# duanzhiihao/myDetection

Hardware: AMD Instinct MI355X
Metric: images/sec at batch 32, 640x640, YOLOv3-80 (backbone -> FPN -> head -> decode -> NMS) (higher is better)
Workload: dtype f32; 1 GPU; yolov3_80 (Darknet-53 + YOLOv3 FPN/head + decode + conf 0.005/top-512/NMS 0.45), batch 32/GPU, 640x640, random-init calibrated weights, hipGraph replay (1 batch lane per GPU); global_batch=32, image_size=640, parallelism=dp1, batch_lanes=1, batch_lanes_rule=model.batch_lanes_hint, passes=153, exchange=none

## Files before the change

include/mydet.h:

```cpp
#ifndef MYDET_H
#define MYDET_H

#include <stdint.h>

#ifdef __cplusplus
extern "C" {
#endif

#define MYDET_ABI_VERSION 2

#define MYDET_E_BADARG   (-1)
#define MYDET_E_UNSUPP   (-2)

#define MYDET_ACT_NONE   0
#define MYDET_ACT_LEAKY  1
#define MYDET_ACT_SWISH  2

int mydet_abi_version(void);

int mydet_conv2d_igemm_f32(const float *x, int64_t ldx, const float *w,
                           const float *scale, const float *shift,
                           const float *residual, int64_t ldr, const float *a_gate,
                           void *workspace, int64_t workspace_bytes,
                           float *y, int64_t ldy,
// ... 36 lines not shown

int mydet_maxpool3s2_f32(const float *x, int64_t ldx, float *y, int64_t ldy, int B, int H, int W, int C,
                         int Ho, int Wo, void *stream);

int mydet_bifpn_fuse_f32(int n, const float *in0, int64_t ld0, int mode0, const float *in1, int64_t ld1, int mode1,
                         const float *in2, int64_t ld2, int mode2, const float *weights, float *y, int64_t ldy,
                         int B, int H, int W, int C, void *stream);

int mydet_upsample_concat_f32(const float *a, int64_t lda, int Ha, int Wa, int C1,
                              const float *b, int64_t ldb, int C2,
                              float *y, int64_t ldy, int B, int Ho, int Wo, void *stream);

int mydet_conv1x1_upcat_f32(const float *x_lo, int64_t ld_lo, int C_lo, const float *x_hi, int64_t ld_hi, int C_hi,
                            const float *w, const float *scale, const float *shift, void *workspace,
                            int64_t workspace_bytes, float *y, int64_t ldy, int B, int H, int W, int Cout, int act,
                            void *stream);

int64_t mydet_split_bf16_elems(int Cout, int K);
int mydet_split_bf16_f32(const float *w, int Cout, int K, uint16_t *planes, void *stream);
int mydet_conv2d_igemm_b3_f32(const float *x, int64_t ldx, const uint16_t *w_planes, const float *scale, const float *shift,
                              const float *residual, int64_t ldr, const float *a_gate, void *workspace, int64_t workspace_bytes, float *y,
                              int64_t ldy, int B, int H, int W, int Cin, int Cout, int KH, int KW, int stride, int pad_t,
                              int pad_l, int Ho, int Wo, int act, void *stream);
int mydet_conv3x3_p3_f32(const float *x, int64_t ldx, const uint16_t *w_planes, const float *scale, const float *shift,
                         const float *residual, int64_t ldr, float *y, int64_t ldy, int B, int H, int W, int Cin, int Cout,
                         int stride, int act, void *stream);
int mydet_conv3x3_p3_plan(int Ho, int Wo, int Cout, int stride, int32_t *out);
int mydet_conv_stem_p3_f32(const float *x, int64_t sxb, int64_t sxc, int64_t sxh, int64_t sxw, const uint16_t *w0_planes,
                           const float *scale0, const float *shift0, int act0, const uint16_t *w1_planes, const float *scale1,
                           const float *shift1, int act1, float *y, int64_t ldy, int B, int H, int W, int C0, int Cout,
                           int stride0, int pad_t, int pad_l, int Hs, int Ws, int stride1, void *stream);
int mydet_conv_stem_p3_lds_bytes(void);
int mydet_conv_b3_reload_tuning(void);

int mydet_conv_igemm_occupancy(int cfg, int *assumed);

int mydet_conv_igemm_plan(int cfg, int B, int Ho, int Wo, int Cin, int Cout, int taps,
                          int64_t workspace_bytes, int cus, int32_t *out);

int mydet_space_to_depth_f32(const float *x, int64_t sb, int64_t sc, int64_t sh, int64_t sw, float *y, int64_t ldy,
                             int B, int C, int H, int W, void *stream);

int mydet_spp_concat_f32(const float *x, int64_t ldx, float *y, int64_t ldy, int B, int H, int W, int C, int k0, int k1,
                         int k2, void *stream);

#define MYDET_DECODE_YOLO   0
#define MYDET_DECODE_RETINA 1
#define MYDET_DECODE_FCOS   2
#define MYDET_DECODE_RAPID  3
typedef struct mydet_decode_level {
    const float *box; int64_t ldbox;
    const float *cls; int64_t ldcls;
    const float *anchors_wh;
    int H, W;
    float stride;
    int64_t n_off;
} mydet_decode_level;
int mydet_decode_levels_f32(int mode, int nlevels, const mydet_decode_level *levels, int box_astride, int box_c0,
                            int cls_astride, int cls_c0, int conf_c0, int A, int C, int B, int img_h, int img_w,
                            float *bbox, int64_t *class_idx, float *score, int64_t N, void *stream);
int mydet_decode_uv5_levels_f32(int nlevels, const mydet_decode_level *levels, int box_astride, int box_c0,
                                int cls_astride, int cls_c0, int conf_c0, int A, int C, int B, int img_h, int img_w,
                                float *bbox, int64_t *class_idx, float *score, int64_t N, void *stream);
int mydet_decode_f32(int mode,
                     const float *box, int64_t ldbox, int box_astride, int box_c0,
                     const float *cls, int64_t ldcls, int cls_astride, int cls_c0, int conf_c0,
// ... 225 lines not shown
```

mydetection_amd/_lib.py:

```python
import ctypes
import os

_HERE = os.path.dirname(os.path.abspath(__file__))
LIB_PATH = os.environ.get('MYDET_LIB_PATH') or os.path.join(_HERE, 'lib', 'libmydet_hip.so')

c_int, c_i64, c_f32, c_f64, c_ptr = ctypes.c_int, ctypes.c_int64, ctypes.c_float, ctypes.c_double, ctypes.c_void_p

SIGNATURES = {
    'mydet_abi_version': [],
    'mydet_conv2d_igemm_f32': [c_ptr, c_i64, c_ptr, c_ptr, c_ptr, c_ptr, c_i64, c_ptr, c_ptr, c_i64, c_ptr, c_i64]
    + [c_int] * 13 + [c_ptr],
    'mydet_wino_weights_floats': [c_int, c_int],
    'mydet_wino_weights_f32': [c_ptr, c_int, c_int, c_ptr, c_ptr],
    'mydet_conv2d_wino_f32': [c_ptr, c_i64, c_ptr, c_ptr, c_ptr, c_ptr, c_i64, c_ptr, c_i64, c_ptr, c_i64] + [c_int] * 6
    + [c_ptr],
    'mydet_wino_plan': [c_int] * 5 + [c_i64, c_int, c_ptr],
    'mydet_wino4_weights_floats': [c_int, c_int],
    'mydet_wino4_weights_f32': [c_ptr, c_int, c_int, c_ptr, c_ptr],
    'mydet_wino4_workspace_bytes': [c_int, c_int, c_int, c_int, c_int],
    'mydet_wino4_reload_tuning': [],
    'mydet_conv_b3_reload_tuning': [],
    'mydet_conv_igemm_occupancy': [c_int, c_ptr],
    'mydet_conv_igemm_plan': [c_int] * 7 + [c_i64, c_int, c_ptr],
    'mydet_split_bf16_elems': [c_int, c_int],
    'mydet_split_bf16_f32': [c_ptr, c_int, c_int, c_ptr, c_ptr],
    'mydet_conv2d_igemm_b3_f32': [c_ptr, c_i64, c_ptr, c_ptr, c_ptr, c_ptr, c_i64, c_ptr, c_ptr, c_i64, c_ptr, c_i64] + [c_int] * 13 + [c_ptr],
    'mydet_conv3x3_p3_f32': [c_ptr, c_i64, c_ptr, c_ptr, c_ptr, c_ptr, c_i64, c_ptr, c_i64] + [c_int] * 7 + [c_ptr],
    'mydet_conv3x3_p3_plan': [c_int, c_int, c_int, c_int, c_ptr],
    'mydet_conv_stem_p3_f32': [c_ptr, c_i64, c_i64, c_i64, c_i64, c_ptr, c_ptr, c_ptr, c_int, c_ptr, c_ptr, c_ptr, c_int, c_ptr, c_i64]
    + [c_int] * 11 + [c_ptr],
    'mydet_conv_stem_p3_lds_bytes': [],
    'mydet_wino4_tail_plan': [c_int, c_int, c_int, c_int, c_int, c_int, c_ptr],
    'mydet_conv2d_wino4_f32': [c_ptr, c_i64, c_ptr, c_ptr, c_ptr, c_ptr, c_i64, c_ptr, c_i64, c_ptr, c_i64] + [c_int] * 6 + [c_ptr],
    'mydet_dwconv_slices': [c_int, c_int, c_int, c_int, c_int],
    'mydet_dwconv_se_groups': [c_int, c_int, c_int, c_int, c_int],
    'mydet_dwconv_f32': [c_ptr, c_i64, c_ptr, c_ptr, c_ptr, c_ptr, c_i64] + [c_int] * 11 + [c_ptr, c_int, c_ptr, c_ptr],
    'mydet_channel_sums_f32': [c_ptr, c_i64, c_int, c_int, c_int, c_int, c_ptr, c_int, c_ptr],
    'mydet_se_gate_f32': [c_ptr, c_int, c_int, c_int, c_int, c_ptr, c_ptr, c_int, c_ptr, c_ptr, c_ptr, c_ptr],
    'mydet_maxpool3s2_f32': [c_ptr, c_i64, c_ptr, c_i64] + [c_int] * 6 + [c_ptr],
    'mydet_bifpn_fuse_f32': [c_int, c_ptr, c_i64, c_int, c_ptr, c_i64, c_int, c_ptr, c_i64, c_int, c_ptr, c_ptr, c_i64,
                             c_int, c_int, c_int, c_int, c_ptr],
    'mydet_conv2d_stem_f32': [c_ptr, c_i64, c_i64, c_i64, c_i64, c_ptr, c_ptr, c_ptr, c_ptr, c_i64] + [c_int] * 10 + [c_ptr],
    'mydet_upsample_concat_f32': [c_ptr, c_i64, c_int, c_int, c_int, c_ptr, c_i64, c_int, c_ptr, c_i64, c_int, c_int,
                                  c_int, c_ptr],
    'mydet_conv1x1_upcat_f32': [c_ptr, c_i64, c_int, c_ptr, c_i64, c_int, c_ptr, c_ptr, c_ptr, c_ptr, c_i64, c_ptr, c_i64]
    + [c_int] * 5 + [c_ptr],
    'mydet_space_to_depth_f32': [c_ptr, c_i64, c_i64, c_i64, c_i64, c_ptr, c_i64, c_int, c_int, c_int, c_int, c_ptr],
    'mydet_spp_concat_f32': [c_ptr, c_i64, c_ptr, c_i64] + [c_int] * 7 + [c_ptr],
    'mydet_decode_levels_f32': [c_int, c_int, c_ptr, c_int, c_int, c_int, c_int, c_int, c_int, c_int, c_int, c_int, c_int,
                                c_ptr, c_ptr, c_ptr, c_i64, c_ptr],
    'mydet_decode_uv5_levels_f32': [c_int, c_ptr, c_int, c_int, c_int, c_int, c_int, c_int, c_int, c_int, c_int, c_int,
                                    c_ptr, c_ptr, c_ptr, c_i64, c_ptr],
    'mydet_decode_f32': [c_int, c_ptr, c_i64, c_int, c_int, c_ptr, c_i64, c_int, c_int, c_int, c_ptr, c_int, c_int,
                         c_int, c_int, c_int, c_f32, c_int, c_int, c_ptr, c_ptr, c_ptr, c_i64, c_i64, c_ptr],
# ... 168 lines not shown
```

mydetection_amd/csrc/common.h:

```cpp
#pragma once
#include <hip/hip_runtime.h>
#include <stdint.h>

#include "mydet.h"

typedef float f32x4 __attribute__((ext_vector_type(4)));
typedef float f32x16 __attribute__((ext_vector_type(16)));

#define MYDET_WAVE 64

static inline int mydet_launch_status() { return (int)hipGetLastError(); }

static inline int mydet_cu_count() {
    static int n = 0;
    if (n == 0) {
        int dev = 0, v = 0;
        if (hipGetDevice(&dev) == hipSuccess && hipDeviceGetAttribute(&v, hipDeviceAttributeMultiprocessorCount, dev) == hipSuccess && v > 0)
            n = v;
        else
            n = 256;
    }
    return n;
}

// ... 24 lines not shown
    return __builtin_amdgcn_rcpf(1.0f + __builtin_amdgcn_exp2f(t));
}

__device__ __forceinline__ float mydet_act(float v, int act) {
    if (act == MYDET_ACT_LEAKY) return v > 0.0f ? v : v * 0.1f;
    if (act == MYDET_ACT_SWISH) return v * mydet_sigmoid_fast(v);
    return v;
}

__device__ __forceinline__ void mydet_lds_barrier() {
    __builtin_amdgcn_fence(__ATOMIC_RELEASE, "workgroup", "local");
    __builtin_amdgcn_s_barrier();
    __builtin_amdgcn_fence(__ATOMIC_ACQUIRE, "workgroup", "local");
}

__device__ __forceinline__ __amdgpu_buffer_rsrc_t mydet_rsrc(const void *base, int64_t bytes) {
    const uint64_t a = (uint64_t)base;
    const unsigned lo = __builtin_amdgcn_readfirstlane((unsigned)a);
    const unsigned hi = __builtin_amdgcn_readfirstlane((unsigned)(a >> 32));
    const int64_t capped = bytes > 0x7FFFFFF0ll ? 0x7FFFFFF0ll : bytes;
    const int n = __builtin_amdgcn_readfirstlane((int)capped);
    return __builtin_amdgcn_make_buffer_rsrc((void *)(((uint64_t)hi << 32) | lo), 0, n, 0x00020000);
}

__device__ __forceinline__ int mydet_xcd_remap(int bid, int nblk) {
    const int xcd = bid & 7, q = nblk >> 3, r = nblk & 7;
    const int base = xcd < r ? xcd * (q + 1) : r * (q + 1) + (xcd - r) * q;
    return base + (bid >> 3);
}

int mydet_pw_skinny(const float *x, int64_t ldx, const float *w, const float *scale, const float *shift,
                    const float *residual, int64_t ldr, const float *gate, float *y, int64_t ldy, int B, int HW, int Cin,
                    int Cout, int act, void *stream);
```

mydetection_amd/csrc/conv_igemm.hip:

```cpp
#include <cstdlib>

#include "common.h"
#include "split_bf16.h"

namespace {

constexpr unsigned OOB = 0xFFFFFFFFu;

struct ConvArgs {
    const float *x, *w, *scale, *shift, *res, *gate;
    float *y;
    int64_t ldx, ldr, ldy;
    int B, H, W, Cin, Cout, KH, KW, stride, pad_t, pad_l, Ho, Wo, act;
    int M, K, ntiles, nblk;
    int tile0, splits;
    float *ws;
    size_t ws_bytes;
    const float *x1;
    int64_t ldx1;
    int C1;
    const unsigned short *wsplit;
};

typedef unsigned u32x4 __attribute__((ext_vector_type(4)));

__device__ __forceinline__ f32x4 buf_load16(__amdgpu_buffer_rsrc_t rsrc, unsigned voff) {
    return __builtin_bit_cast(f32x4, __builtin_amdgcn_raw_buffer_load_b128(rsrc, voff, 0, 0));
}

template <int ACT, bool RES, bool FULL, int TM, int TN>
__device__ __forceinline__ void epilogue(const ConvArgs &p, f32x16 (&acc)[TM][TN], int m_base, int n_base,
                                         int fr, int fh, const float (&pscl)[TN], const float (&psft)[TN]) {
    const __amdgpu_buffer_rsrc_t yr = mydet_rsrc(p.y, (int64_t)p.M * p.ldy * 4);
    const __amdgpu_buffer_rsrc_t rr = mydet_rsrc(RES ? p.res : p.y, (int64_t)p.M * (RES ? p.ldr : p.ldy) * 4);
    const unsigned ldy4 = (unsigned)p.ldy * 4u, ldr4 = (unsigned)p.ldr * 4u;
#pragma unroll
    for (int j = 0; j < TN; ++j) {
        const int n = n_base + j * 32 + fr;
        const bool nok = FULL || n < p.Cout;
        const float scl = pscl[j], sft = psft[j];
#pragma unroll
        for (int i = 0; i < TM; ++i) {
            const int mrow = m_base + i * 32 + 4 * fh;
            const unsigned ybase = (unsigned)mrow * ldy4 + (unsigned)n * 4u;
            const unsigned rbase = (unsigned)mrow * ldr4 + (unsigned)n * 4u;
            float rv[16];
            if (RES) {
#pragma unroll
                for (int r = 0; r < 16; ++r) {
                    const int dr = (r & 3) + 8 * (r >> 2);
                    const bool ok = FULL || (nok && mrow + dr < p.M);
                    rv[r] = __builtin_bit_cast(float, __builtin_amdgcn_raw_buffer_load_b32(
                                                          rr, ok ? rbase + (unsigned)dr * ldr4 : OOB, 0, 0));
                }
            }
#pragma unroll
            for (int r = 0; r < 16; ++r) {
                const int dr = (r & 3) + 8 * (r >> 2);
                float v = acc[i][j][r] * scl + sft;
                if (ACT == MYDET_ACT_LEAKY) v = v > 0.0f ? v : v * 0.1f;
                if (ACT == MYDET_ACT_SWISH) v = v * mydet_sigmoid_fast(v);
                if (RES) v += rv[r];
                const bool ok = FULL || (nok && mrow + dr < p.M);
                __builtin_amdgcn_raw_buffer_store_b32(__builtin_bit_cast(unsigned, v), yr,
                                                      ok ? ybase + (unsigned)dr * ldy4 : OOB, 0, 0);
            }
        }
    }
}

template <int BM, int BN, int WM, int WN, int BK, bool CIN32, int ACT, bool RES, bool GATE, bool SPLIT = false, bool CAT = false>
__global__ __launch_bounds__(WM * WN * 64) void conv_igemm_kernel(const ConvArgs p) {
    constexpr int NT = WM * WN * 64;
#ifndef IGEMM_PF
#define IGEMM_PF 2
#endif
    constexpr int PF = IGEMM_PF;
    constexpr int LDS_LD = BK + 4;
    constexpr int CH = BK / 4;
    constexpr int RP = NT / CH;
    constexpr int TM = BM / (WM * 32), TN = BN / (WN * 32);
    constexpr int AI = BM / RP, BI = BN / RP;
    static_assert(BM % RP == 0 && BN % RP == 0, "tile rows must fill whole staging passes");
    extern __shared__ __attribute__((aligned(16))) float smem[];
    float *As = smem;
    float *Bs = smem + 2 * BM * LDS_LD;

    const int tid = threadIdx.x;
    const int lid = SPLIT ? p.tile0 + (int)blockIdx.x / p.splits : mydet_xcd_remap(blockIdx.x, p.nblk);
    const int m0 = (lid / p.ntiles) * BM;
    const int n0 = (lid % p.ntiles) * BN;

    const int hwo = p.Ho * p.Wo;
    const int b0 = m0 / hwo;
    const int64_t img = (int64_t)p.H * p.W * p.ldx;
    const __amdgpu_buffer_rsrc_t xr = mydet_rsrc(p.x + b0 * img, (p.B - b0) * img * 4);
    const __amdgpu_buffer_rsrc_t wr = mydet_rsrc(p.w, (int64_t)p.Cout * p.K * 4);
    const int64_t img1 = (int64_t)(p.H >> 1) * (p.W >> 1) * p.ldx1;
    const __amdgpu_buffer_rsrc_t xr1 = mydet_rsrc(CAT ? p.x1 + b0 * img1 : p.w, CAT ? (p.B - b0) * img1 * 4 : 16);
    const __amdgpu_buffer_rsrc_t gr = mydet_rsrc(GATE ? p.gate : p.w, (int64_t)p.B * p.Cin * 4);

// ... 970 lines not shown
        out[4] = pl.split ? pl.total - pl.rem : pl.total;
        out[5] = pl.split ? pl.rem : 0;
        out[6] = pl.split ? pl.splits : 1;
        return 0;
    });
}

extern "C" int64_t mydet_split_bf16_elems(int Cout, int K) {
    if (Cout <= 0 || K <= 0 || (K & 3)) return 0;
    return (int64_t)((K + 15) >> 4) * 3 * ((Cout + B3_COUT_PAD - 1) / B3_COUT_PAD * B3_COUT_PAD) * 16;
}

extern "C" int mydet_split_bf16_f32(const float *w, int Cout, int K, uint16_t *planes, void *stream) {
    if (!w || !planes || Cout <= 0 || K <= 0) return MYDET_E_BADARG;
    if (K & 3) return MYDET_E_UNSUPP;
    const int CoutP = (Cout + B3_COUT_PAD - 1) / B3_COUT_PAD * B3_COUT_PAD;
    const int64_t total = (int64_t)((K + 15) >> 4) * CoutP * 16;
    if ((total + 255) / 256 > 0x7fffffff) return MYDET_E_UNSUPP;
    hipLaunchKernelGGL(split_bf16_kernel, dim3((unsigned)((total + 255) / 256)), dim3(256), 0, (hipStream_t)stream, w, Cout, K,
                       CoutP, planes);
    return mydet_launch_status();
}

static int g_b3_form = -1;
static int b3_form() {
    if (g_b3_form < 0) {
        const char *w = getenv("MYDET_B3_WIDE"), *v = getenv("MYDET_B3_WAVES");
        g_b3_form = ((w && *w == '1') ? 1 : 0) | ((v && atoi(v) == 8) ? 2 : 0);
    }
    return g_b3_form;
}
extern "C" int mydet_conv_b3_reload_tuning(void) {
    g_b3_form = -1;
    return b3_form();
}

extern "C" int mydet_conv2d_igemm_b3_f32(const float *x, int64_t ldx, const uint16_t *w_planes, const float *scale,
                                         const float *shift, const float *residual, int64_t ldr, const float *a_gate, void *workspace,
                                         int64_t workspace_bytes, float *y, int64_t ldy, int B, int H, int W, int Cin, int Cout,
                                         int KH, int KW, int stride, int pad_t, int pad_l, int Ho, int Wo, int act, void *stream) {
    if (!x || !w_planes || !y || B <= 0 || H <= 0 || W <= 0 || Cin <= 0 || Cout <= 0 || KH <= 0 || KW <= 0 || stride <= 0 ||
        Ho <= 0 || Wo <= 0)
        return MYDET_E_BADARG;
    if ((ldx & 3) || ldx < Cin || ldy < Cout || (residual && ldr < Cout)) return MYDET_E_BADARG;
    if (((uintptr_t)x & 15) || ((uintptr_t)w_planes & 15) || ((uintptr_t)y & 15) || (residual && ((uintptr_t)residual & 15)) ||
        (scale && ((uintptr_t)scale & 15)) || (shift && ((uintptr_t)shift & 15)))
        return MYDET_E_BADARG;
    if (act < 0 || act > 2) return MYDET_E_BADARG;
    if (a_gate && (KH != 1 || KW != 1 || ((uintptr_t)a_gate & 15))) return MYDET_E_BADARG;
    if (((Cin & 15) && !(KH == 1 && KW == 1 && !(Cin & 3))) || (ldy & 3) || (residual && (ldr & 3))) return MYDET_E_UNSUPP;
    if ((Cin & 15) && (Cout > 192 ? b3_form() & 1 : 0)) return MYDET_E_UNSUPP;
    const int64_t M64 = (int64_t)B * Ho * Wo, K64 = (int64_t)KH * KW * Cin;
    if (M64 > (int64_t)1 << 30 || K64 > (int64_t)1 << 30) return MYDET_E_BADARG;
    const int64_t img_bytes = (int64_t)H * W * ldx * 4;
    const int64_t span_imgs = 256 / ((int64_t)Ho * Wo) + 2;
    if (M64 * ldy * 4 >= 0x7FFFFFF0ll || (residual && M64 * ldr * 4 >= 0x7FFFFFF0ll)) return MYDET_E_UNSUPP;
    if (KH * KW > 31 || img_bytes * span_imgs >= 0x7FFFFFF0ll || mydet_split_bf16_elems(Cout, (int)K64) * 2 >= 0x7FFFFFF0ll) return MYDET_E_UNSUPP;
    ConvArgs a;
    a.x = x; a.w = nullptr; a.scale = scale; a.shift = shift; a.res = residual; a.gate = a_gate; a.y = y;
    a.ldx = ldx; a.ldr = ldr; a.ldy = ldy;
    a.B = B; a.H = H; a.W = W; a.Cin = Cin; a.Cout = Cout; a.KH = KH; a.KW = KW; a.stride = stride;
    a.pad_t = pad_t; a.pad_l = pad_l; a.Ho = Ho; a.Wo = Wo; a.act = act;
    a.M = (int)M64; a.K = (int)K64; a.ntiles = 0; a.nblk = 0; a.tile0 = 0; a.splits = 1;
    a.x1 = nullptr; a.ldx1 = 0; a.C1 = 0; a.wsplit = w_planes;
    a.ws = ((uintptr_t)workspace & 15) ? nullptr : (float *)workspace;
    a.ws_bytes = workspace_bytes > 0 ? (size_t)workspace_bytes : 0;
    if (Cout <= 64) return launch_b3<128, 64>(a, (hipStream_t)stream);
    static const int half_tiles = [] { const char *e = getenv("MYDET_B3_HALF_TILES"); return e ? atoi(e) : mydet_cu_count() / 2; }();
    if (((M64 + 127) / 128) * ((Cout + 127) / 128) <= half_tiles) return launch_b3<64, 128>(a, (hipStream_t)stream);
    const int form = a_gate ? 0 : b3_form();
    if ((form & 1) && Cout > 192) return launch_b3w(a, (hipStream_t)stream);
    if (form & 2) return launch_b3<128, 128, 4>(a, (hipStream_t)stream);
    return launch_b3<128, 128>(a, (hipStream_t)stream);
}

extern "C" int mydet_conv_igemm_occupancy(int cfg, int *assumed) {
    int n = 0, as = 0;
    hipError_t e = hipErrorInvalidValue;
#define MYDET_OCC(BM, BN, WM, WN, BK, PER_CU)                                                                                       \
    {                                                                                                                                \
        auto kern = &conv_igemm_kernel<BM, BN, WM, WN, BK, true, MYDET_ACT_LEAKY, false, false, false, false>;                        \
        const size_t lds = (size_t)2 * (BM + BN) * (BK + 4) * sizeof(float);                                                          \
        static unsigned long long m = 0;                                                                                             \
        if (const int rc = mydet_lds_opt_in(m, kern, (int)lds)) return rc;                                                            \
        e = hipOccupancyMaxActiveBlocksPerMultiprocessor(&n, kern, WM * WN * 64, lds);                                                \
        as = PER_CU;                                                                                                                 \
    }
    switch (cfg) {
        case 0: MYDET_OCC(128, 128, 2, 2, 32, 2) break;
        case 1: MYDET_OCC(128, 64, 2, 2, 32, 2) break;
        case 2: MYDET_OCC(128, 32, 4, 1, 32, 3) break;
        case 3: MYDET_OCC(64, 64, 2, 2, 32, 4) break;
        case 6: MYDET_OCC(128, 64, 2, 2, 16, cfg6_per_cu()) break;
        case 9: MYDET_OCC(128, 96, 4, 1, 32, 2) break;
        case 8: MYDET_OCC(128, 128, 2, 4, 32, 2) break;
        default: return MYDET_E_BADARG;
    }
#undef MYDET_OCC
    if (assumed) *assumed = as;
// ... 35 lines not shown
```

mydetection_amd/ops.py:

```python
import collections
import ctypes
import functools
import math
import os
import threading

import numpy as np
import torch

from . import _lib

ACT_NONE, ACT_LEAKY, ACT_SWISH = 0, 1, 2
DECODE_YOLO, DECODE_RETINA, DECODE_FCOS, DECODE_RAPID = 0, 1, 2, 3
TOPK = 512


def _stream():
    return ctypes.c_void_p(torch.cuda.current_stream().cuda_stream)


class KernelTimer:

    def __init__(self, chain=False):
        self.spans = {}
# ... 179 lines not shown

WINOGRAD4 = os.environ.get('MYDET_CONV_WINO4', '1') != '0'
WINO4_MIN_CIN = int(os.environ.get('MYDET_WINO4_MIN_CIN', '64'))
WINO4_MIN_ITEMS = int(os.environ.get('MYDET_WINO4_MIN_ITEMS', '512'))


def wino4_items(B, H, W, Cout):
    return -(-(B * -(-H // 4) * -(-W // 4)) // 32) * -(-Cout // 32)


def wino4_weights(w_ohwi):
    require_gpu(w_ohwi, 'wino4_weights')
    Cout, kh, kw, Cin = w_ohwi.shape
    if kh != 3 or kw != 3 or Cout % 4:
        return None
    n = _lib.lib().mydet_wino4_weights_floats(Cout, Cin)
    if n <= 0:
        return None
    u = torch.empty(n, dtype=torch.float32, device=w_ohwi.device)
    w = w_ohwi.contiguous()
    _lib.check(_lib.lib().mydet_wino4_weights_f32(_ptr(w), Cout, Cin, _ptr(u), _stream()), 'mydet_wino4_weights_f32')
    return u


SPLIT_BF16 = os.environ.get('MYDET_CONV_SPLIT_BF16', '1') != '0'


B3_MIN_ROWS = int(os.environ.get('MYDET_B3_MIN_ROWS', '8192'))
B3_MIN_FLOP = float(os.environ.get('MYDET_B3_MIN_FLOP', '3e9'))
B3_KPAD = os.environ.get('MYDET_B3_KPAD', '1') != '0'
B3_EXPAND_MIN_ROWS = int(os.environ.get('MYDET_B3_EXPAND_MIN_ROWS', '3000'))
B3_GATED_MIN_COUT = int(os.environ.get('MYDET_B3_GATED_MIN_COUT', '64'))
B3_GATED_MIN_ROWS = int(os.environ.get('MYDET_B3_GATED_MIN_ROWS', '3000'))


def b3_takes(M, Cin, Cout, k, min_rows=None, min_cout=128):
    if not SPLIT_BF16 or not (k > 1 or Cout >= min_cout):
        return False
    if Cin % 16 and not (B3_KPAD and k == 1 and Cin % 4 == 0):
        return False
    if min_rows is not None:
        return M >= min_rows
    return M >= B3_MIN_ROWS and 2.0 * M * k * k * Cin * Cout >= B3_MIN_FLOP


CONV_P3 = os.environ.get('MYDET_CONV_P3', '1') != '0'
P3_MIN_WGS = int(os.environ.get('MYDET_P3_MIN_WGS', '512'))
P3_S1_MAX_CIN = int(os.environ.get('MYDET_P3_S1_MAX_CIN', '32'))
P3_MIN_FILL = float(os.environ.get('MYDET_P3_MIN_FILL', '0.75'))

P3Plan = collections.namedtuple('P3Plan', 'bn strip tx_n ty_n main_tiles tiles_img ntn lds')


@functools.lru_cache(maxsize=None)
def p3_plan(Ho, Wo, Cout, stride):
    out = (ctypes.c_int32 * 8)()
    _lib.check(_lib.lib().mydet_conv3x3_p3_plan(Ho, Wo, Cout, stride, out), 'mydet_conv3x3_p3_plan')
    return P3Plan(*out)


def p3_tiles(Ho, Wo, stride):
    return p3_plan(Ho, Wo, 64, stride).tiles_img


def p3_takes(B, Ho, Wo, Cin, Cout, k, stride, pad):
    if not (CONV_P3 and SPLIT_BF16) or k != 3 or stride not in (1, 2) or tuple(pad) != (1, 1, 1, 1) or Cin % 16:
# ... 38 lines not shown
    if residual is not None:
        residual, ldr = to_nhwc(residual)
        assert residual.shape == out.shape
    if b3 is not None and gate is None and act in (ACT_NONE, ACT_LEAKY) and p3_takes(B, Ho, Wo, Cin, Cout, k, stride, pad):
        y = conv3x3_p3(x, b3, scale, shift, stride, act, residual=residual, out=out, cout=Cout)
        if y is not None:
            return y
    if (wino4 is not None and WINOGRAD and WINOGRAD4 and gate is None and k == 3 and stride == 1 and tuple(pad) == (1, 1, 1, 1)
            and ldy % 4 == 0 and ldr % 4 == 0 and (wino is None or wino4_items(B, H, W, Cout) >= WINO4_MIN_ITEMS)):
        ws = wino4_workspace(x.device, _lib.lib().mydet_wino4_workspace_bytes(B, H, W, Cin, Cout))
        t0 = TIMER.start() if TIMER else None
        code = _lib.lib().mydet_conv2d_wino4_f32(_ptr(x), ldx, _ptr(wino4), _ptr(scale), _ptr(shift), _ptr(residual), ldr,
                                                 _ptr(ws), ws.numel() * 4, _ptr(out), ldy, B, H, W, Cin, Cout, act, _stream())
        if t0:
            name = f'conv_wino4 {Cin}->{Cout} k3s1 {H}x{W}' if TIMER_DETAIL else 'conv_wino4'
            TIMER.stop(name, t0, 2.0 * B * Ho * Wo * Cout * 9 * Cin,
                       4.0 * (B * H * W * Cin + B * Ho * Wo * Cout * (2 if residual is not None else 1) + 9 * Cin * Cout))
        _lib.check(code, 'mydet_conv2d_wino4_f32')
        return out
    if (wino is not None and WINOGRAD and gate is None and k == 3 and stride == 1 and tuple(pad) == (1, 1, 1, 1)
            and ldy % 4 == 0 and ldr % 4 == 0):
        ws = conv_workspace(x.device)
        t0 = TIMER.start() if TIMER else None
        code = _lib.lib().mydet_conv2d_wino_f32(_ptr(x), ldx, _ptr(wino), _ptr(scale), _ptr(shift), _ptr(residual), ldr,
                                                _ptr(ws), ws.numel() * 4, _ptr(out), ldy, B, H, W, Cin, Cout, act,
                                                _stream())
        if t0:
            name = f'conv_wino {Cin}->{Cout} k3s1 {H}x{W}' if TIMER_DETAIL else 'conv_wino'
            TIMER.stop(name, t0, 2.0 * B * Ho * Wo * Cout * 9 * Cin,
                       4.0 * (B * H * W * Cin + B * Ho * Wo * Cout * (2 if residual is not None else 1) + 9 * Cin * Cout))
        _lib.check(code, 'mydet_conv2d_wino_f32')
        return out
    ws = conv_workspace(x.device)
    if (b3 is not None and b3_takes(B * Ho * Wo, Cin, Cout, k, b3_min_rows, min_cout=B3_GATED_MIN_COUT if gate is not None else 128)
            and (gate is None or (k == 1 and act == ACT_NONE))):
        t0 = TIMER.start() if TIMER else None
        code = _lib.lib().mydet_conv2d_igemm_b3_f32(
            _ptr(x), ldx, _ptr(b3), _ptr(scale), _ptr(shift), _ptr(residual), ldr, _ptr(gate), _ptr(ws), ws.numel() * 4, _ptr(out), ldy,
            B, H, W, Cin, Cout, k, k, stride, pad[0], pad[1], Ho, Wo, act, _stream())
        if code != -2:
            if t0:
                name = f'conv_igemm_b3 {Cin}->{Cout} k{k}s{stride} {H}x{W}' if TIMER_DETAIL else 'conv_igemm_b3'
                b_in, b_out = 4.0 * B * H * W * Cin, 4.0 * B * Ho * Wo * Cout
                b_rest = 4.0 * (k * k * Cin * Cout) + (b_out if residual is not None else 0.0)
                TIMER.stop(name, t0, 2.0 * B * Ho * Wo * Cout * k * k * Cin, b_in + b_out + b_rest)
            _lib.check(code, 'mydet_conv2d_igemm_b3_f32')
            return out
    t0 = TIMER.start() if TIMER else None
    code = _lib.lib().mydet_conv2d_igemm_f32(
        _ptr(x), ldx, _ptr(w_ohwi), _ptr(scale), _ptr(shift), _ptr(residual), ldr, _ptr(gate),
        _ptr(ws), ws.numel() * 4 if ws is not None else 0, _ptr(out), ldy,
        B, H, W, Cin, Cout, k, k, stride, pad[0], pad[1], Ho, Wo, act, _stream())
    if t0:
        name = f'conv_igemm {Cin}->{Cout} k{k}s{stride} {H}x{W}' if TIMER_DETAIL else 'conv_igemm'
        b_in, b_out = 4.0 * B * H * W * Cin, 4.0 * B * Ho * Wo * Cout
        b_rest = 4.0 * (k * k * Cin * Cout) + (b_out if residual is not None else 0.0)
        TIMER.stop(name, t0, 2.0 * B * Ho * Wo * Cout * k * k * Cin, b_in + b_out + b_rest,
                   (0.0 if interior == 'in' else b_in) + (0.0 if interior == 'out' else b_out) + b_rest)
    _lib.check(code, 'mydet_conv2d_igemm_f32')
    return out


def conv3x3_p3(x, b3, scale, shift, stride, act, residual=None, out=None, out_ld=None, cout=None):
    require_gpu(x, 'conv3x3_p3')
    x, ldx = to_nhwc(x)
    B, Cin, H, W = x.shape
    Cout = int(cout if cout is not None else (shift if shift is not None else scale).shape[0])
# ... 1523 lines not shown
```

Measured before the change: 1688 images/sec.

## Add dedicated pointwise split-bf16 conv kernel with DMA-to-LDS pipeline

Adds a specialised 1x1 stride-1 convolution kernel for the three-plane bf16 split path. It streams activation and weight tiles straight into LDS with buffer-load-to-LDS, multi-buffers them, and shares the epilogue through a new header. A heuristic decides per layer whether to use it instead of the generic implicit-GEMM b3 kernel, and it also lowers the minimum Cout so 64-channel pointwise layers can use the b3 path. This is meant to cut im2col and indexing overhead and improve latency hiding on 1x1 layers, at the cost of more kernel variants and a routing heuristic that may choose badly for some shapes.

```diff
diff --git a/include/mydet.h b/include/mydet.h
--- a/include/mydet.h
+++ b/include/mydet.h
@@ -92,6 +92,8 @@
                            int stride0, int pad_t, int pad_l, int Hs, int Ws, int stride1, void *stream);
 int mydet_conv_stem_p3_lds_bytes(void);
 int mydet_conv_b3_reload_tuning(void);
+
+int mydet_conv_pw_b3_takes(int64_t M, int Cin, int Cout, int64_t ldx, int64_t ldy, int64_t ldr, int act, int has_gate);
 
 int mydet_conv_igemm_occupancy(int cfg, int *assumed);
 
diff --git a/mydetection_amd/_lib.py b/mydetection_amd/_lib.py
--- a/mydetection_amd/_lib.py
+++ b/mydetection_amd/_lib.py
@@ -20,6 +20,7 @@
     'mydet_wino4_workspace_bytes': [c_int, c_int, c_int, c_int, c_int],
     'mydet_wino4_reload_tuning': [],
     'mydet_conv_b3_reload_tuning': [],
+    'mydet_conv_pw_b3_takes': [c_i64, c_int, c_int, c_i64, c_i64, c_i64, c_int, c_int],
     'mydet_conv_igemm_occupancy': [c_int, c_ptr],
     'mydet_conv_igemm_plan': [c_int] * 7 + [c_i64, c_int, c_ptr],
     'mydet_split_bf16_elems': [c_int, c_int],
diff --git a/mydetection_amd/csrc/common.h b/mydetection_amd/csrc/common.h
--- a/mydetection_amd/csrc/common.h
+++ b/mydetection_amd/csrc/common.h
@@ -80,3 +80,7 @@
 int mydet_pw_skinny(const float *x, int64_t ldx, const float *w, const float *scale, const float *shift,
                     const float *residual, int64_t ldr, const float *gate, float *y, int64_t ldy, int B, int HW, int Cin,
                     int Cout, int act, void *stream);
+
+int mydet_conv_pw_b3(const float *x, int64_t ldx, const uint16_t *w_planes, const float *scale, const float *shift,
+                     const float *residual, int64_t ldr, float *y, int64_t ldy, int64_t M, int Cin, int Cout, int act, void *stream);
+int mydet_pw_b3_reload(void);
diff --git a/mydetection_amd/csrc/conv_epilogue.h b/mydetection_amd/csrc/conv_epilogue.h
--- /dev/null
+++ b/mydetection_amd/csrc/conv_epilogue.h
@@ -0,0 +1,49 @@
+#pragma once
+#include "common.h"
+
+namespace {
+
+constexpr unsigned OOB = 0xFFFFFFFFu;
+
+template <int ACT, bool RES, bool FULL, int TM, int TN, class Args>
+__device__ __forceinline__ void epilogue(const Args &p, f32x16 (&acc)[TM][TN], int m_base, int n_base,
+                                         int fr, int fh, const float (&pscl)[TN], const float (&psft)[TN]) {
+    const __amdgpu_buffer_rsrc_t yr = mydet_rsrc(p.y, (int64_t)p.M * p.ldy * 4);
+    const __amdgpu_buffer_rsrc_t rr = mydet_rsrc(RES ? p.res : p.y, (int64_t)p.M * (RES ? p.ldr : p.ldy) * 4);
+    const unsigned ldy4 = (unsigned)p.ldy * 4u, ldr4 = (unsigned)p.ldr * 4u;
+#pragma unroll
+    for (int j = 0; j < TN; ++j) {
+        const int n = n_base + j * 32 + fr;
+        const bool nok = FULL || n < p.Cout;
+        const float scl = pscl[j], sft = psft[j];
+#pragma unroll
+        for (int i = 0; i < TM; ++i) {
+            const int mrow = m_base + i * 32 + 4 * fh;
+            const unsigned ybase = (unsigned)mrow * ldy4 + (unsigned)n * 4u;
+            const unsigned rbase = (unsigned)mrow * ldr4 + (unsigned)n * 4u;
+            float rv[16];
+            if (RES) {
+#pragma unroll
+                for (int r = 0; r < 16; ++r) {
+                    const int dr = (r & 3) + 8 * (r >> 2);
+                    const bool ok = FULL || (nok && mrow + dr < p.M);
+                    rv[r] = __builtin_bit_cast(float, __builtin_amdgcn_raw_buffer_load_b32(
+                                                          rr, ok ? rbase + (unsigned)dr * ldr4 : OOB, 0, 0));
+                }
+            }
+#pragma unroll
+            for (int r = 0; r < 16; ++r) {
+                const int dr = (r & 3) + 8 * (r >> 2);
+                float v = acc[i][j][r] * scl + sft;
+                if (ACT == MYDET_ACT_LEAKY) v = v > 0.0f ? v : v * 0.1f;
+                if (ACT == MYDET_ACT_SWISH) v = v * mydet_sigmoid_fast(v);
+                if (RES) v += rv[r];
+                const bool ok = FULL || (nok && mrow + dr < p.M);
+                __builtin_amdgcn_raw_buffer_store_b32(__builtin_bit_cast(unsigned, v), yr,
+                                                      ok ? ybase + (unsigned)dr * ldy4 : OOB, 0, 0);
+            }
+        }
+    }
+}
+
+}
diff --git a/mydetection_amd/csrc/conv_igemm.hip b/mydetection_amd/csrc/conv_igemm.hip
--- a/mydetection_amd/csrc/conv_igemm.hip
+++ b/mydetection_amd/csrc/conv_igemm.hip
@@ -1,11 +1,10 @@
 #include <cstdlib>
 
 #include "common.h"
+#include "conv_epilogue.h"
 #include "split_bf16.h"
 
 namespace {
-
-constexpr unsigned OOB = 0xFFFFFFFFu;
 
 struct ConvArgs {
     const float *x, *w, *scale, *shift, *res, *gate;
@@ -26,47 +25,6 @@
 
 __device__ __forceinline__ f32x4 buf_load16(__amdgpu_buffer_rsrc_t rsrc, unsigned voff) {
     return __builtin_bit_cast(f32x4, __builtin_amdgcn_raw_buffer_load_b128(rsrc, voff, 0, 0));
-}
-
-template <int ACT, bool RES, bool FULL, int TM, int TN>
-__device__ __forceinline__ void epilogue(const ConvArgs &p, f32x16 (&acc)[TM][TN], int m_base, int n_base,
-                                         int fr, int fh, const float (&pscl)[TN], const float (&psft)[TN]) {
-    const __amdgpu_buffer_rsrc_t yr = mydet_rsrc(p.y, (int64_t)p.M * p.ldy * 4);
-    const __amdgpu_buffer_rsrc_t rr = mydet_rsrc(RES ? p.res : p.y, (int64_t)p.M * (RES ? p.ldr : p.ldy) * 4);
-    const unsigned ldy4 = (unsigned)p.ldy * 4u, ldr4 = (unsigned)p.ldr * 4u;
-#pragma unroll
-    for (int j = 0; j < TN; ++j) {
-        const int n = n_base + j * 32 + fr;
-        const bool nok = FULL || n < p.Cout;
-        const float scl = pscl[j], sft = psft[j];
-#pragma unroll
-        for (int i = 0; i < TM; ++i) {
-            const int mrow = m_base + i * 32 + 4 * fh;
-            const unsigned ybase = (unsigned)mrow * ldy4 + (unsigned)n * 4u;
-            const unsigned rbase = (unsigned)mrow * ldr4 + (unsigned)n * 4u;
-            float rv[16];
-            if (RES) {
-#pragma unroll
-                for (int r = 0; r < 16; ++r) {
-                    const int dr = (r & 3) + 8 * (r >> 2);
-                    const bool ok = FULL || (nok && mrow + dr < p.M);
-                    rv[r] = __builtin_bit_cast(float, __builtin_amdgcn_raw_buffer_load_b32(
-                                                          rr, ok ? rbase + (unsigned)dr * ldr4 : OOB, 0, 0));
-                }
-            }
-#pragma unroll
-            for (int r = 0; r < 16; ++r) {
-                const int dr = (r & 3) + 8 * (r >> 2);
-                float v = acc[i][j][r] * scl + sft;
-                if (ACT == MYDET_ACT_LEAKY) v = v > 0.0f ? v : v * 0.1f;
-                if (ACT == MYDET_ACT_SWISH) v = v * mydet_sigmoid_fast(v);
-                if (RES) v += rv[r];
-                const bool ok = FULL || (nok && mrow + dr < p.M);
-                __builtin_amdgcn_raw_buffer_store_b32(__builtin_bit_cast(unsigned, v), yr,
-                                                      ok ? ybase + (unsigned)dr * ldy4 : OOB, 0, 0);
-            }
-        }
-    }
 }
 
 template <int BM, int BN, int WM, int WN, int BK, bool CIN32, int ACT, bool RES, bool GATE, bool SPLIT = false, bool CAT = false>
@@ -1103,6 +1061,7 @@
 }
 extern "C" int mydet_conv_b3_reload_tuning(void) {
     g_b3_form = -1;
+    mydet_pw_b3_reload();
     return b3_form();
 }
 
@@ -1136,6 +1095,9 @@
     a.x1 = nullptr; a.ldx1 = 0; a.C1 = 0; a.wsplit = w_planes;
     a.ws = ((uintptr_t)workspace & 15) ? nullptr : (float *)workspace;
     a.ws_bytes = workspace_bytes > 0 ? (size_t)workspace_bytes : 0;
+    if (KH == 1 && KW == 1 && stride == 1 && pad_t == 0 && pad_l == 0 && Ho == H && Wo == W &&
+        mydet_conv_pw_b3_takes(M64, Cin, Cout, ldx, ldy, residual ? ldr : 0, act, a_gate != nullptr))
+        return mydet_conv_pw_b3(x, ldx, w_planes, scale, shift, residual, ldr, y, ldy, M64, Cin, Cout, act, stream);
     if (Cout <= 64) return launch_b3<128, 64>(a, (hipStream_t)stream);
     static const int half_tiles = [] { const char *e = getenv("MYDET_B3_HALF_TILES"); return e ? atoi(e) : mydet_cu_count() / 2; }();
     if (((M64 + 127) / 128) * ((Cout + 127) / 128) <= half_tiles) return launch_b3<64, 128>(a, (hipStream_t)stream);
diff --git a/mydetection_amd/csrc/conv_pw_b3.hip b/mydetection_amd/csrc/conv_pw_b3.hip
--- /dev/null
+++ b/mydetection_amd/csrc/conv_pw_b3.hip
@@ -0,0 +1,219 @@
+#include <cstdlib>
+
+#include "common.h"
+#include "conv_epilogue.h"
+#include "split_bf16.h"
+
+namespace {
+
+constexpr int PW_COUT_PAD = 256;
+__device__ __forceinline__ int pw_b3_unit(int rr, int h) { return 2 * rr + (h ^ ((rr >> 2) & 1)); }
+
+struct PwArgs {
+    const float *x, *scale, *shift, *res;
+    const unsigned short *wsplit;
+    float *y;
+    int64_t ldx, ldr, ldy;
+    int M, Cin, Cout, ntiles, nblk;
+};
+
+typedef __attribute__((address_space(3))) void *lds_ptr;
+
+template <int BN, int RA, int ACT, bool RES>
+__global__ __launch_bounds__(256, 2) void conv_pw_b3_kernel(const PwArgs p) {
+    constexpr int NW = 4, BM = NW * 32, TN = BN / 32;
+    constexpr int A_BYTES = BM * 128;
+    constexpr int B_PIECES = 2 * 3 * TN;
+    constexpr int BPW = B_PIECES / NW;
+    constexpr int B_BYTES = B_PIECES * 1024;
+    static_assert(B_PIECES % NW == 0 && (RA == 2 || RA == 3), "every wave issues the same number of requests");
+    extern __shared__ __attribute__((aligned(16))) char smem_pw[];
+
+    const int tid = threadIdx.x;
+    const int wave = __builtin_amdgcn_readfirstlane(tid >> 6), lane = tid & 63;
+    const int lid = mydet_xcd_remap(blockIdx.x, p.nblk);
+    const int m0 = (lid / p.ntiles) * BM;
+    const int n0 = (lid % p.ntiles) * BN;
+    const int rows = p.M - m0 < BM ? p.M - m0 : BM;
+    const __amdgpu_buffer_rsrc_t xr = mydet_rsrc(p.x + (int64_t)m0 * p.ldx, ((int64_t)(rows - 1) * p.ldx + p.Cin) * 4);
+    const int CoutP = (p.Cout + PW_COUT_PAD - 1) / PW_COUT_PAD * PW_COUT_PAD;
+    const int nk16 = (p.Cin + 15) >> 4;
+    const __amdgpu_buffer_rsrc_t wr = mydet_rsrc(p.wsplit, (int64_t)nk16 * 3 * CoutP * 32);
+    const unsigned plane_bytes = (unsigned)CoutP * 32u, slab_bytes = 3u * plane_bytes;
+
+    unsigned aoff[4];
+    int achan[4];
+#pragma unroll
+    for (int i = 0; i < 4; ++i) {
+        const int r = (wave * 4 + i) * 8 + (lane >> 3);
+        const int c = (lane & 7) ^ ((r >> 1) & 7);
+        aoff[i] = r < rows ? (unsigned)r * (unsigned)p.ldx * 4u + (unsigned)c * 16u : OOB;
+        achan[i] = c * 4;
+    }
+    const unsigned bsrc = (unsigned)(n0 * 32 + pw_b3_unit(((lane >> 5) << 4) | (lane & 15), (lane >> 4) & 1) * 16);
+    auto dma_a = [&](int kt, int slot) {
+        char *st = smem_pw + slot * A_BYTES;
+        const int k0 = kt * 32;
+#pragma unroll
+        for (int i = 0; i < 4; ++i) {
+            const bool ok = aoff[i] != OOB && k0 + achan[i] < p.Cin;
+            __builtin_amdgcn_raw_ptr_buffer_load_lds(xr, (lds_ptr)(st + (wave * 4 + i) * 1024), 16,
+                                                     ok ? aoff[i] + (unsigned)k0 * 4u : OOB, 0, 0, 0);
+        }
+    };
+    auto dma_b = [&](int kt, int slot) {
+        char *st = smem_pw + RA * A_BYTES + slot * B_BYTES;
+#pragma unroll
+        for (int i = 0; i < BPW; ++i) {
+            const int idx = wave * BPW + i;
+            const int s = idx / (3 * TN), pl = (idx / TN) % 3, j = idx % TN;
+            const int k16 = 2 * kt + s;
+            __builtin_amdgcn_raw_ptr_buffer_load_lds(
+                wr, (lds_ptr)(st + idx * 1024), 16, k16 < nk16 ? bsrc : OOB,
+                __builtin_amdgcn_readfirstlane((unsigned)k16 * slab_bytes + (unsigned)pl * plane_bytes + (unsigned)j * 1024u), 0, 0);
+        }
+    };
+
+    const int fr = lane & 31, fh = lane >> 5;
+    const int arow = wave * 32 + fr;
+    const int asw = (arow >> 1) & 7;
+    const int a_off = arow * 128;
+    const int b_off = RA * A_BYTES + ((((fr >> 4) * 2 + fh) * 16 + (fr & 15)) * 16);
+    f32x16 acc[1][TN];
+#pragma unroll
+    for (int j = 0; j < TN; ++j)
+#pragma unroll
+        for (int r = 0; r < 16; ++r) acc[0][j][r] = 0.f;
+    float pscl[TN], psft[TN];
+#pragma unroll
+    for (int j = 0; j < TN; ++j) {
+        const int n = n0 + j * 32 + fr;
+        const int nc = n < p.Cout ? n : 0;
+        pscl[j] = p.scale ? p.scale[nc] : 1.0f;
+        psft[j] = p.shift ? p.shift[nc] : 0.0f;
+    }
+    auto compute = [&](int sa, int sb) {
+        const char *sta = smem_pw + sa * A_BYTES + a_off, *stb = smem_pw + sb * B_BYTES + b_off;
+#pragma unroll
+        for (int s = 0; s < 2; ++s) {
+            const int c = 4 * s + 2 * fh;
+            const f32x4 v0 = *reinterpret_cast<const f32x4 *>(sta + ((c ^ asw) * 16));
+            const f32x4 v1 = *reinterpret_cast<const f32x4 *>(sta + (((c + 1) ^ asw) * 16));
+            bf16x4 lo[3], hi[3];
+            split3(v0, lo[0], lo[1], lo[2]);
+            split3(v1, hi[0], hi[1], hi[2]);
+            bf16x8 af[3], bf[TN][3];
+#pragma unroll
+            for (int pl = 0; pl < 3; ++pl) af[pl] = __builtin_shufflevector(lo[pl], hi[pl], 0, 1, 2, 3, 4, 5, 6, 7);
+#pragma unroll
+            for (int j = 0; j < TN; ++j)
+#pragma unroll
+                for (int pl = 0; pl < 3; ++pl)
+                    bf[j][pl] = *reinterpret_cast<const bf16x8 *>(stb + ((s * 3 + pl) * TN + j) * 1024);
+#pragma unroll
+            for (int t = 0; t < 6; ++t)
+#pragma unroll
+                for (int j = 0; j < TN; ++j)
+                    acc[0][j] = __builtin_amdgcn_mfma_f32_32x32x16_bf16(af[SPLIT_PA[t]], bf[j][SPLIT_PB[t]], acc[0][j], 0, 0, 0);
+        }
+    };
+
+    constexpr int WAIT = 0x0070 | (4 * (RA - 2));
+    const int nk = (p.Cin + 31) >> 5;
+    dma_b(0, 0);
+    dma_a(0, 0);
+    if (RA == 3) dma_a(1, 1);
+    __builtin_amdgcn_s_waitcnt(WAIT);
+    __builtin_amdgcn_s_barrier();
+    int sa = 0, sn = RA - 1, sb = 0;
+    for (int kt = 0; kt < nk; ++kt) {
+        dma_b(kt + 1, sb ^ 1);
+        dma_a(kt + RA - 1, sn);
+        compute(sa, sb);
+        __builtin_amdgcn_s_waitcnt(WAIT);
+        __builtin_amdgcn_s_barrier();
+        sa = sa == RA - 1 ? 0 : sa + 1;
+        sn = sn == RA - 1 ? 0 : sn + 1;
+        sb ^= 1;
+    }
+    __builtin_amdgcn_s_waitcnt(0x0070);
+
+    const int m_base = m0 + wave * 32;
+    if ((m0 + BM <= p.M) && (n0 + BN <= p.Cout))
+        epilogue<ACT, RES, true, 1, TN>(p, acc, m_base, n0, fr, fh, pscl, psft);
+    else
+        epilogue<ACT, RES, false, 1, TN>(p, acc, m_base, n0, fr, fh, pscl, psft);
+}
+
+template <int BN, int RA, int ACT, bool RES>
+int launch_pw_inst(const PwArgs &a, hipStream_t stream) {
+    auto kern = &conv_pw_b3_kernel<BN, RA, ACT, RES>;
+    constexpr int lds = RA * 128 * 128 + 2 * 6 * (BN / 32) * 1024;
+    static unsigned long long attr_set = 0;
+    if (const int e = mydet_lds_opt_in(attr_set, kern, lds)) return e;
+    hipLaunchKernelGGL(kern, dim3(a.nblk), dim3(256), lds, stream, a);
+    return mydet_launch_status();
+}
+
+template <int BN, int RA>
+int launch_pw(const PwArgs &a0, int act, hipStream_t stream) {
+    PwArgs a = a0;
+    a.ntiles = (a.Cout + BN - 1) / BN;
+    a.nblk = ((a.M + 127) / 128) * a.ntiles;
+    const bool res = a.res != nullptr;
+    if (act == MYDET_ACT_LEAKY)
+        return res ? launch_pw_inst<BN, RA, MYDET_ACT_LEAKY, true>(a, stream) : launch_pw_inst<BN, RA, MYDET_ACT_LEAKY, false>(a, stream);
+    return res ? launch_pw_inst<BN, RA, MYDET_ACT_NONE, true>(a, stream) : launch_pw_inst<BN, RA, MYDET_ACT_NONE, false>(a, stream);
+}
+
+int g_pw_b3 = -1;
+int pw_b3_mode() {
+    if (g_pw_b3 < 0) {
+        const char *e = getenv("MYDET_PW_B3");
+        const int v = e ? atoi(e) : 1;
+        g_pw_b3 = v < 0 ? 0 : v;
+    }
+    return g_pw_b3;
+}
+
+}
+
+int mydet_pw_b3_reload(void) {
+    g_pw_b3 = -1;
+    return pw_b3_mode();
+}
+
+extern "C" int mydet_conv_pw_b3_takes(int64_t M, int Cin, int Cout, int64_t ldx, int64_t ldy, int64_t ldr, int act, int has_gate) {
+    const int mode = pw_b3_mode();
+    if (!mode || has_gate || (act != MYDET_ACT_NONE && act != MYDET_ACT_LEAKY)) return 0;
+    if (M <= 0 || M > (int64_t)1 << 30 || Cin <= 0 || Cout <= 0 || (Cin & 3) || (ldx & 3) || ldx < Cin || (ldy & 3) || ldy < Cout ||
+        (ldr && ((ldr & 3) || ldr < Cout)))
+        return 0;
+    if (ldx * 4 * 128 >= 0x7FFFFFF0ll) return 0;
+    const int cus = mydet_cu_count(), slots = 2 * cus;
+    const int64_t mtiles = (M + 127) / 128;
+    const bool half = Cout > 64 && mtiles * ((Cout + 127) / 128) <= cus / 2;
+    const int BN = Cout <= 64 ? 64 : 128;
+    const int64_t total = (half ? (M + 63) / 64 : mtiles) * ((Cout + BN - 1) / BN);
+    const int nk = (Cin + 15) / 16;
+    const int64_t rounds = total / slots, rem = total % slots;
+    int64_t splits = rem > 0 ? slots / rem : 0;
+    if (splits > 16) splits = 16;
+    if (splits > nk / 8) splits = nk / 8;
+    const bool small = rounds == 0 && total * 4 <= slots && nk >= 32;
+    if (rem > 0 && splits >= 2 && (small || (nk >= 64 && rounds >= 2 && rounds <= 4 && rem * 2 <= slots))) return 0;
+    if (mode >= 2) return 1;
+    if (half) return 0;
+    if (Cout > 64 && Cout <= 128 && Cin <= 256 && total > slots) return 0;
+    return 1;
+}
+
+int mydet_conv_pw_b3(const float *x, int64_t ldx, const uint16_t *w_planes, const float *scale, const float *shift,
+                     const float *residual, int64_t ldr, float *y, int64_t ldy, int64_t M, int Cin, int Cout, int act, void *stream) {
+    if (!mydet_conv_pw_b3_takes(M, Cin, Cout, ldx, ldy, residual ? ldr : 0, act, 0)) return MYDET_E_UNSUPP;
+    PwArgs a;
+    a.x = x; a.scale = scale; a.shift = shift; a.res = residual; a.wsplit = w_planes; a.y = y;
+    a.ldx = ldx; a.ldr = residual ? ldr : 0; a.ldy = ldy;
+    a.M = (int)M; a.Cin = Cin; a.Cout = Cout; a.ntiles = 0; a.nblk = 0;
+    return Cout <= 64 ? launch_pw<64, 3>(a, act, (hipStream_t)stream) : launch_pw<128, 2>(a, act, (hipStream_t)stream);
+}
diff --git a/mydetection_amd/ops.py b/mydetection_amd/ops.py
--- a/mydetection_amd/ops.py
+++ b/mydetection_amd/ops.py
@@ -235,6 +235,7 @@
 B3_EXPAND_MIN_ROWS = int(os.environ.get('MYDET_B3_EXPAND_MIN_ROWS', '3000'))
 B3_GATED_MIN_COUT = int(os.environ.get('MYDET_B3_GATED_MIN_COUT', '64'))
 B3_GATED_MIN_ROWS = int(os.environ.get('MYDET_B3_GATED_MIN_ROWS', '3000'))
+B3_PW_MIN_COUT = int(os.environ.get('MYDET_B3_PW_MIN_COUT', '64'))
 
 
 def b3_takes(M, Cin, Cout, k, min_rows=None, min_cout=128):
@@ -339,7 +340,11 @@
         _lib.check(code, 'mydet_conv2d_wino_f32')
         return out
     ws = conv_workspace(x.device)
-    if (b3 is not None and b3_takes(B * Ho * Wo, Cin, Cout, k, b3_min_rows, min_cout=B3_GATED_MIN_COUT if gate is not None else 128)
+    min_cout = B3_GATED_MIN_COUT if gate is not None else 128
+    if (b3 is not None and gate is None and B3_PW_MIN_COUT < 128 and k == 1 and stride == 1 and not any(pad) and
+            _lib.lib().mydet_conv_pw_b3_takes(B * H * W, Cin, Cout, ldx, ldy, ldr, act, 0)):
+        min_cout = B3_PW_MIN_COUT
+    if (b3 is not None and b3_takes(B * Ho * Wo, Cin, Cout, k, b3_min_rows, min_cout=min_cout)
             and (gate is None or (k == 1 and act == ACT_NONE))):
         t0 = TIMER.start() if TIMER else None
         code = _lib.lib().mydet_conv2d_igemm_b3_f32(
```

After: 1699 images/sec, median of 6. No clear change (+0.6%).
